# aquaskyline/Clairvoyante

Hardware: AMD Instinct MI355X
Metric: candidate tensors/sec (higher is better)
Workload: dtype f32

## Files before the change

clairvoyante_amd/csrc/cv_kernels_conv.hpp:

```cpp
#pragma once

template <int P, bool ACT = false>
__device__ __forceinline__ unsigned pool_code4(const f4 (&older)[P > 1 ? P - 1 : 1], f4 v, f4 o)
{
    unsigned c = 0;
#pragma unroll
    for (int r = 0; r < 4; r++) {
        int idx = P - 1;
#pragma unroll
        for (int d = P - 2; d >= 0; d--) {
            bool hit = older[d][r] == o[r];
            if constexpr (ACT) hit = hit && __builtin_signbit(older[d][r]) == __builtin_signbit(o[r]);
            idx = hit ? d : idx;
        }
        (void)v;
        c |= (unsigned)idx << (4 * r);
    }
    return c;
}

template <int POOL, bool SAVE = false>
__global__ __launch_bounds__(256) void conv1_tm(const float *__restrict__ x, int64_t n,
                                                 const float *__restrict__ wp1,
                                                 const float *__restrict__ bias, int cout,
                                                 f4 *__restrict__ out_tm, int G, u32x2 *__restrict__ code_tm = nullptr)
{
    constexpr int HIN = CV_INPUT_H, HOUT = HIN - POOL + 1, SPLIT = 4;
    const int lane = threadIdx.x & 63;
    const int wv = blockIdx.x * 4 + (threadIdx.x >> 6);
    const int g = wv / SPLIT, part = wv % SPLIT;
    if (g >= G) return;
    const int r0 = (HOUT * part) / SPLIT, r1 = (HOUT * (part + 1)) / SPLIT;
    const int c = lane & 15, q = lane >> 4;
    int64_t cand = (int64_t)g * 16 + c;
    if (cand >= n) cand = n - 1;
    const float *xp = x + (size_t)cand * (HIN * 16) + q;
    float A[4];
#pragma unroll
    for (int kw = 0; kw < 4; kw++) A[kw] = wp1[kw * 64 + lane];
    const f4 b4 = load_bias4(bias, 0, q, cout);
    f4 pw[POOL > 1 ? POOL - 1 : 1][4];
#pragma unroll
    for (int j = 0; j < (POOL > 1 ? POOL - 1 : 1); j++)
#pragma unroll
        for (int w = 0; w < 4; w++) pw[j][w] = (f4){0.f, 0.f, 0.f, 0.f};
    float xw[4], xn[4];
#pragma unroll
    for (int w = 0; w < 4; w++) xw[w] = xp[r0 * 16 + w * 4];
    f4 *op = out_tm + (size_t)g * HOUT * 4 * 64 + lane;
    const int hend = r1 + POOL - 1;
#pragma unroll 1
    for (int h = r0; h < hend; h++) {
        {
            const int hn = h + 1 < hend ? h + 1 : h;
#pragma unroll
            for (int w = 0; w < 4; w++) xn[w] = xp[hn * 16 + w * 4];
        }
        f4 acc[4];
#pragma unroll
        for (int w = 0; w < 4; w++) acc[w] = (f4){0.f, 0.f, 0.f, 0.f};
#pragma unroll
        for (int kw = 0; kw < 4; kw++)
#pragma unroll
            for (int wo = 0; wo < 4; wo++) {
                const int wi = wo + kw - 1;
                if (wi < 0 || wi > 3) continue;
                acc[wo] = mfma4(A[kw], xw[wi], acc[wo]);
            }
        if constexpr (!SAVE && POOL > 1) {
#pragma unroll
            for (int w = 0; w < 4; w++) {
                const f4 t = acc[w] + b4;
                const f4 o = max4(pw[POOL - 2][w], t);
#pragma unroll
                for (int j = POOL - 2; j > 0; j--) pw[j][w] = max4(pw[j - 1][w], t);
                pw[0][w] = t;
                if (h - r0 >= POOL - 1) op[(size_t)((h - (POOL - 1)) * 4 + w) * 64] = selu4(o);
            }
#pragma unroll
            for (int w = 0; w < 4; w++) xw[w] = xn[w];
            continue;
        }
        f4 v[4];
#pragma unroll
        for (int w = 0; w < 4; w++) v[w] = selu4(acc[w] + b4);
        if constexpr (POOL > 1) {
            f4 o[4];
#pragma unroll
            for (int w = 0; w < 4; w++) {
                o[w] = v[w];
#pragma unroll
                for (int j = 0; j < POOL - 1; j++) o[w] = max4(o[w], pw[j][w]);
            }
            if constexpr (SAVE) {
                if (h - r0 >= POOL - 1) {
                    unsigned cw[4];
#pragma unroll
                    for (int w = 0; w < 4; w++) {
                        f4 older[POOL - 1];
#pragma unroll
                        for (int j = 0; j < POOL - 1; j++) older[j] = pw[j][w];
                        cw[w] = pool_code4<POOL, true>(older, v[w], o[w]);
                    }
                    code_tm[((size_t)g * HOUT + (h - (POOL - 1))) * 64 + lane] = (u32x2){cw[0] | (cw[1] << 16), cw[2] | (cw[3] << 16)};
                }
            }
#pragma unroll
            for (int j = 0; j + 1 < POOL - 1; j++)
#pragma unroll
                for (int w = 0; w < 4; w++) pw[j][w] = pw[j + 1][w];
#pragma unroll
            for (int w = 0; w < 4; w++) pw[POOL - 2][w] = v[w];
            if (h - r0 >= POOL - 1) {
#pragma unroll
                for (int w = 0; w < 4; w++) op[(size_t)((h - (POOL - 1)) * 4 + w) * 64] = o[w];
            }
        } else {
#pragma unroll
            for (int w = 0; w < 4; w++) op[(size_t)(h * 4 + w) * 64] = v[w];
        }
#pragma unroll
        for (int w = 0; w < 4; w++) xw[w] = xn[w];
    }
}

__device__ __forceinline__ f4 selu4_low(f4 v)
{
    const cvm::f2v a = cvm::selu2((cvm::f2v){v[0], v[1]});
    return (f4){a[0], a[1], 0.0f, 0.0f};
}

template <int FRONT, bool HALF = false>
struct front_source {
    static constexpr int NP = FRONT > 1 ? FRONT - 1 : 1;
    const float *xp;
    float A[4];
    f4 b4;
    f4 cw[NP][4];
    float xc[4], xn[4];
    int hx;

    __device__ __forceinline__ void load_x(float (&dst)[4], int h)
    {
        if (h < CV_INPUT_H) {
#pragma unroll
            for (int w = 0; w < 4; w++) dst[w] = xp[h * 16 + w * 4];
        }
    }
    __device__ __forceinline__ void conv1_row(f4 (&v)[4])
    {
        f4 acc[4];
#pragma unroll
        for (int w = 0; w < 4; w++) acc[w] = (f4){0.f, 0.f, 0.f, 0.f};
#pragma unroll
        for (int kw = 0; kw < 4; kw++)
#pragma unroll
            for (int wo = 0; wo < 4; wo++) {
                const int wi = wo + kw - 1;
                if (wi < 0 || wi > 3) continue;
                acc[wo] = mfma4(A[kw], xc[wi], acc[wo]);
            }
#pragma unroll
        for (int w = 0; w < 4; w++) v[w] = acc[w] + b4;
#pragma unroll
        for (int w = 0; w < 4; w++) xc[w] = xn[w];
        hx++;
        load_x(xn, hx + 1);
    }
    __device__ __forceinline__ void init(const float *x, int64_t cand, int q, const float *wp1,
                                         const float *bias1, int cout1, int lane, int h0 = 0)
    {
        xp = x + (size_t)cand * (CV_INPUT_H * 16) + q;
#pragma unroll
        for (int kw = 0; kw < 4; kw++) A[kw] = wp1[kw * 64 + lane];
        b4 = load_bias4(bias1, 0, q, cout1);
        hx = h0;
        load_x(xc, h0);
        load_x(xn, h0 + 1);
        if constexpr (FRONT > 1) {
#pragma unroll
            for (int r = 0; r < FRONT - 1; r++) {
                f4 v[4];
                conv1_row(v);
#pragma unroll
                for (int w = 0; w < 4; w++) {
#pragma unroll
                    for (int j = FRONT - 2; j > 0; j--) cw[j][w] = r == 0 ? v[w] : max4(cw[j - 1][w], v[w]);
                    cw[0][w] = v[w];
                }
            }
        }
    }
    __device__ __forceinline__ void next(f4 (&row)[4][1])
    {
        f4 v[4];
        conv1_row(v);
        if constexpr (FRONT > 1) {
#pragma unroll
            for (int w = 0; w < 4; w++) {
                const f4 o = max4(cw[FRONT - 2][w], v[w]);
#pragma unroll
                for (int j = FRONT - 2; j > 0; j--) cw[j][w] = max4(cw[j - 1][w], v[w]);
                cw[0][w] = v[w];
                row[w][0] = HALF ? selu4_low(o) : selu4(o);
            }
        } else {
#pragma unroll
            for (int w = 0; w < 4; w++) row[w][0] = HALF ? selu4_low(v[w]) : selu4(v[w]);
        }
    }
};

#define CV_CONV_XCD_UNITS(W) ((W) != 1 && (W) != 2 && (W) != 4)
template <int KH, int CINB, int NT, int POOL, int HIN, int FRONT, int MODE, int HSPLIT = 1, int KS4 = 4>
__global__ __launch_bounds__(256, 2) void conv_tm(const f4 *__restrict__ in_tm, const float *__restrict__ x,
                                                   int64_t n, const float *__restrict__ wp1,
                                                   const float *__restrict__ bias1, int cout1,
                                                   const f4 *__restrict__ wp, const float *__restrict__ bias,
                                                   int cout, f4 *__restrict__ out_tm, f4 *__restrict__ act_tm, int G,
                                                   int rows_per = 0)
{
    static_assert(FRONT == 0 || CINB == 1, "the fused first layer feeds one 16-channel fragment");
    static_assert(MODE != 2 || (POOL == 1 && FRONT == 0), "the data-gradient pass has no pooling / first layer");
    static_assert(HSPLIT >= 1 || FRONT == 0, "flat ranges read their rows from a TM buffer (position parts may make them: front_source::init h0)");
    static_assert(HSPLIT != 0 || (FRONT == 0 && (MODE != 0 || POOL == 1)), "flat ranges: training kernels, and inference layers without pooling (slim small passes)");
    extern __shared__ __attribute__((aligned(16))) f4 ldsw[];
    constexpr int PADT = MODE == 2 ? KH - 1 - (KH - 1) / 2 : (KH - 1) / 2;
    constexpr int PADL = MODE == 2 ? 2 : 1;
    constexpr int HOUT = HIN - POOL + 1;
    constexpr int NFRAG = NT * KH * 4 * CINB;
    for (int i = threadIdx.x; i < NFRAG * 64; i += 256) ldsw[i] = wp[i];
    __syncthreads();
    const int lane = threadIdx.x & 63;
    int wv = __builtin_amdgcn_readfirstlane(blockIdx.x * 4 + (threadIdx.x >> 6));
    if constexpr (HSPLIT >= 1 && CV_CONV_XCD_UNITS(NT * HSPLIT)) {
        if (gridDim.x >= 16) {
            const int x = blockIdx.x & 7;
            const int lw = __builtin_amdgcn_readfirstlane((blockIdx.x >> 3) * 4 + (threadIdx.x >> 6));
            wv = ((lw / (NT * HSPLIT)) * 8 + x) * (NT * HSPLIT) + lw % (NT * HSPLIT);
        }
    }
    constexpr int HSD = HSPLIT > 0 ? HSPLIT : 1;
    int nt, gF, gL, hs = 0, r0 = 0, r1 = 0;
    if constexpr (HSPLIT == 0) {
        nt = wv % NT;
        r0 = (wv / NT) * rows_per;
        r1 = r0 + rows_per < G * HOUT ? r0 + rows_per : G * HOUT;
        if (r0 >= r1) return;
        gF = r0 / HOUT; gL = (r1 - 1) / HOUT;
    } else {
        const int gt = wv / HSD;
        hs = wv % HSD; nt = gt % NT; gF = gL = gt / NT;
        if (gF >= G) return;
    }
    CV_STAMP_BEGIN
    const int q = lane >> 4;
    const f4 b4 = MODE == 2 ? (f4){0.f, 0.f, 0.f, 0.f} : load_bias4(bias, nt, q, cout);
    const f4 *wl = ldsw + (size_t)nt * (KH * 4 * CINB * 64) + lane;
#pragma unroll 1
    for (int g = gF; g <= gL; g++) {
    int hbeg, hend;
    if constexpr (HSPLIT == 0) {
        const int oa = r0 - g * HOUT > 0 ? r0 - g * HOUT : 0, ob = r1 - g * HOUT < HOUT ? r1 - g * HOUT : HOUT;
        hbeg = oa; hend = POOL > 1 ? ob + POOL - 1 : ob;
    } else {
        hbeg = POOL > 1 ? HOUT * hs / HSD : HIN * hs / HSD;
        hend = POOL > 1 ? HOUT * (hs + 1) / HSD + POOL - 1 : HIN * (hs + 1) / HSD;
    }
    const f4 *inp = in_tm + (size_t)g * (HIN * 4 * CINB * 64) + lane;
    f4 *op = out_tm + (size_t)g * (HOUT * 4 * NT * 64) + (size_t)nt * 64 + lane;

    front_source<FRONT, (KS4 <= 2)> fs;
    if constexpr (FRONT > 0) {
        int64_t cand = (int64_t)g * 16 + (lane & 15);
        if (cand >= n) cand = n - 1;
        fs.init(x, cand, q, wp1, bias1, cout1, lane, hbeg - PADT > 0 ? hbeg - PADT : 0);
    }
    auto fetch_row = [&](int hr, f4 (&row)[4][CINB]) {
        if constexpr (FRONT > 0) {
            fs.next(row);
        } else {
#pragma unroll
            for (int w = 0; w < 4; w++)
#pragma unroll
                for (int cb = 0; cb < CINB; cb++) row[w][cb] = inp[(size_t)((hr * 4 + w) * CINB + cb) * 64];
        }
    };
    constexpr bool SPREAD = FRONT == 0;
    static_assert(CINB <= 3, "the counted wait below names at most 12 fragments");
    const f4 *const inp_s = in_tm + (size_t)__builtin_amdgcn_readfirstlane(g) * (HIN * 4 * CINB * 64);
    const unsigned lane16 = (unsigned)lane * 16u;
    auto load_piece = [&](int hr, int w, int cb, f4 &dst) {
        const f4 *ps = inp_s + (size_t)((hr * 4 + w) * CINB + cb) * 64;
        asm volatile("global_load_dwordx4 %0, %1, %2" : "=v"(dst) : "v"(lane16), "s"(ps));
    };

    f4 win[KH][4][CINB];
    f4 nxt[4][CINB];
    f4 pw[POOL > 1 ? POOL - 1 : 1][4];
    const f4 zero = (f4){0.f, 0.f, 0.f, 0.f};
#pragma unroll
    for (int j = 0; j < (POOL > 1 ? POOL - 1 : 1); j++)
#pragma unroll
        for (int w = 0; w < 4; w++) pw[j][w] = zero;
#pragma unroll
    for (int j = 0; j < KH; j++) {
        const int hr = hbeg + j - PADT;
        f4 tmp[4][CINB];
#pragma unroll
        for (int w = 0; w < 4; w++)
#pragma unroll
            for (int cb = 0; cb < CINB; cb++) tmp[w][cb] = zero;
        if (hr >= 0 && hr < HIN) fetch_row(hr, tmp);
#pragma unroll
        for (int w = 0; w < 4; w++)
#pragma unroll
            for (int cb = 0; cb < CINB; cb++) {
                if (j < KH - 1) win[j][w][cb] = tmp[w][cb]; else nxt[w][cb] = tmp[w][cb];
            }
    }
#pragma unroll 1
    for (int h = hbeg; h < hend; h++) {
#pragma unroll
        for (int w = 0; w < 4; w++)
#pragma unroll
            for (int cb = 0; cb < CINB; cb++) win[KH - 1][w][cb] = nxt[w][cb];
        {
            const int hr = h + 1 + (KH - 1) - PADT;
            if (!SPREAD && hr < HIN) fetch_row(hr, nxt);
        }
        const int hnext = h + 1 + (KH - 1) - PADT < HIN ? h + 1 + (KH - 1) - PADT : HIN - 1;
        f4 acc[4];
#pragma unroll
        for (int w = 0; w < 4; w++) acc[w] = zero;
#pragma unroll
        for (int kh = 0; kh < KH; kh++) {
            const int hr = h + kh - PADT;
            const bool on = hr >= 0 && hr < HIN;
            if (on) {
#pragma unroll
                for (int kw = 0; kw < 4; kw++)
#pragma unroll
                    for (int cb = 0; cb < CINB; cb++) {
                        const f4 A = wl[(size_t)((kh * 4 + kw) * CINB + cb) * 64];
#pragma unroll
                        for (int s = 0; s < KS4; s++)
#pragma unroll
                            for (int wo = 0; wo < 4; wo++) {
                                const int wi = wo + kw - PADL;
                                if (wi < 0 || wi > 3) continue;
                                acc[wo] = mfma4(A[s], win[kh][wi][cb][s], acc[wo]);
                            }
                        if constexpr (SPREAD) {
                            if (kh == 0) load_piece(hnext, kw, cb, nxt[kw][cb]);
                        }
                    }
            } else if (SPREAD && kh == 0) {
#pragma unroll
                for (int kw = 0; kw < 4; kw++)
#pragma unroll
                    for (int cb = 0; cb < CINB; cb++) load_piece(hnext, kw, cb, nxt[kw][cb]);
            }
        }
        if constexpr (SPREAD) {
            {
                if constexpr (CINB == 1)
                    asm volatile("s_waitcnt vmcnt(0)" : "+v"(nxt[0][0]), "+v"(nxt[1][0]), "+v"(nxt[2][0]), "+v"(nxt[3][0]) : : "memory");
                else if constexpr (CINB == 2)
                    asm volatile("s_waitcnt vmcnt(0)" : "+v"(nxt[0][0]), "+v"(nxt[1][0]), "+v"(nxt[2][0]), "+v"(nxt[3][0]),
                                 "+v"(nxt[0][1]), "+v"(nxt[1][1]), "+v"(nxt[2][1]), "+v"(nxt[3][1]) : : "memory");
                else
                    asm volatile("s_waitcnt vmcnt(0)" : "+v"(nxt[0][0]), "+v"(nxt[1][0]), "+v"(nxt[2][0]), "+v"(nxt[3][0]),
                                 "+v"(nxt[0][1]), "+v"(nxt[1][1]), "+v"(nxt[2][1]), "+v"(nxt[3][1]),
                                 "+v"(nxt[0][CINB - 1]), "+v"(nxt[1][CINB - 1]), "+v"(nxt[2][CINB - 1]), "+v"(nxt[3][CINB - 1]) : : "memory");
            }
        }
        if constexpr (MODE == 0 && POOL > 1) {
#pragma unroll
            for (int w = 0; w < 4; w++) {
                const f4 t = acc[w] + b4;
                const f4 o = max4(pw[POOL - 2][w], t);
#pragma unroll
                for (int j = POOL - 2; j > 0; j--) pw[j][w] = max4(pw[j - 1][w], t);
                pw[0][w] = t;
                if (h - hbeg >= POOL - 1) {
                    op[(size_t)((h - (POOL - 1)) * 4 + w) * (NT * 64)] = selu4(o);
                }
            }
#pragma unroll
            for (int j = 0; j + 1 < KH; j++)
#pragma unroll
                for (int w = 0; w < 4; w++)
#pragma unroll
                    for (int cb = 0; cb < CINB; cb++) win[j][w][cb] = win[j + 1][w][cb];
            continue;
        }
        f4 v[4];
        if constexpr (MODE == 2) {
#pragma unroll
            for (int w = 0; w < 4; w++) v[w] = acc[w];
            if (act_tm) {
                const f4 *yp = act_tm + (size_t)g * (HOUT * 4 * NT * 64) + (size_t)nt * 64 + lane;
#pragma unroll
                for (int w = 0; w < 4; w++) {
                    const f4 y = yp[(size_t)(h * 4 + w) * (NT * 64)];
#pragma unroll
                    for (int k = 0; k < 4; k++) v[w][k] *= cv_selu_grad_from_out(y[k]);
                }
            }
        } else {
#pragma unroll
            for (int w = 0; w < 4; w++) v[w] = selu4(acc[w] + b4);
        }
        if constexpr (POOL > 1) {
            f4 o[4];
#pragma unroll
            for (int w = 0; w < 4; w++) {
                o[w] = v[w];
#pragma unroll
                for (int j = 0; j < POOL - 1; j++) o[w] = max4(o[w], pw[j][w]);
            }
            if constexpr (MODE == 1) {
                if (h - hbeg >= POOL - 1) {
                    unsigned cw[4];
#pragma unroll
                    for (int w = 0; w < 4; w++) {
                        f4 older[POOL - 1];
#pragma unroll
                        for (int j = 0; j < POOL - 1; j++) older[j] = pw[j][w];
                        cw[w] = pool_code4<POOL, true>(older, v[w], o[w]);
                    }
                    u32x2 *cp = reinterpret_cast<u32x2 *>(act_tm);
                    cp[(((size_t)g * HOUT + (h - (POOL - 1))) * NT + nt) * 64 + lane] = (u32x2){cw[0] | (cw[1] << 16), cw[2] | (cw[3] << 16)};
                }
            }
#pragma unroll
            for (int j = 0; j + 1 < POOL - 1; j++)
#pragma unroll
                for (int w = 0; w < 4; w++) pw[j][w] = pw[j + 1][w];
#pragma unroll
            for (int w = 0; w < 4; w++) pw[POOL - 2][w] = v[w];
            if (h - hbeg >= POOL - 1) {
#pragma unroll
                for (int w = 0; w < 4; w++) op[(size_t)((h - (POOL - 1)) * 4 + w) * (NT * 64)] = o[w];
            }
        } else {
#pragma unroll
            for (int w = 0; w < 4; w++) op[(size_t)(h * 4 + w) * (NT * 64)] = v[w];
        }
#pragma unroll
        for (int j = 0; j + 1 < KH; j++)
#pragma unroll
            for (int w = 0; w < 4; w++)
#pragma unroll
                for (int cb = 0; cb < CINB; cb++) win[j][w][cb] = win[j + 1][w][cb];
    }
    }
    CV_STAMP_END(MODE == 2 && KH == 3 && CINB == 3, 2);
    CV_STAMP_END(MODE == 1 && KH == 2 && CINB == 1 && FRONT == 0, 6);
}

template <int CH, bool FLAT = false>
__global__ __launch_bounds__(FLAT ? 128 : 256, 2) void front2_tm(const float *__restrict__ x, int64_t n,
                                                     const float *__restrict__ wp1, const float *__restrict__ bias1,
                                                     int cout1, const f4 *__restrict__ wp,
                                                     const float *__restrict__ bias, int cout,
                                                     f4 *__restrict__ out_tm, int G, int rows_per = 0)
{
    constexpr int P1 = 5, H1 = CV_INPUT_H - P1 + 1;
    constexpr int NT = 2, P2 = 4, H2 = H1 - P2 + 1;
    constexpr int NW = NT * 2 * 4 * 64;
    extern __shared__ __attribute__((aligned(16))) f4 lds[];
    f4 *rows = lds + NW;
    for (int i = threadIdx.x; i < NW; i += (FLAT ? 128 : 256)) lds[i] = wp[i];
    const int lane = threadIdx.x & 63, wid = threadIdx.x >> 6;
    const int gl = FLAT ? 0 : wid >> 1, nt = wid & 1;
    int gF, gL, r0 = 0, r1 = 0;
    bool live = true;
    if constexpr (FLAT) {
        r0 = (int)blockIdx.x * rows_per;
        r1 = r0 + rows_per < G * H2 ? r0 + rows_per : G * H2;
        if (r0 >= r1) return;
        gF = r0 / H2; gL = (r1 - 1) / H2;
    } else {
        const int gq = blockIdx.x * 2 + gl;
        live = gq < G;
        gF = gL = live ? gq : G - 1;
    }
    const int q = lane >> 4;
    float A1[4];
#pragma unroll
    for (int kw = 0; kw < 4; kw++) A1[kw] = wp1[kw * 64 + lane];
    const f4 b1 = load_bias4(bias1, 0, q, cout1);
    const f4 b2 = load_bias4(bias, nt, q, cout);
    const f4 *wl = lds + (size_t)nt * (2 * 4 * 64) + lane;
    f4 *myrows = rows + (size_t)gl * (CH * 4 * 64) + lane;
    const f4 zero = (f4){0.f, 0.f, 0.f, 0.f};
    f4 prev[4], m1[4], m2[4], m3[4];
#pragma unroll
    for (int w = 0; w < 4; w++) { prev[w] = zero; m1[w] = zero; m2[w] = zero; m3[w] = zero; }
    __syncthreads();
    CV_PHASE_BEGIN
#pragma unroll 1
    for (int g = gF; g <= gL; g++) {
    int oa = 0, ob = H2;
    if constexpr (FLAT) {
        oa = r0 - g * H2 > 0 ? r0 - g * H2 : 0;
        ob = r1 - g * H2 < H2 ? r1 - g * H2 : H2;
    }
    const int pend = ob + P2 < H1 ? ob + P2 : H1;
    int64_t cand = (int64_t)g * 16 + (lane & 15);
    if (cand >= n) cand = n - 1;
    const float *xp = x + (size_t)cand * (CV_INPUT_H * 16) + q;
    f4 *op = out_tm + (size_t)g * (H2 * 4 * NT * 64) + (size_t)nt * 64 + lane;

    auto out_row = [&](int h, const f4 (&cur)[4], bool has_cur) {
        f4 acc[4];
#pragma unroll
        for (int w = 0; w < 4; w++) acc[w] = zero;
#pragma unroll
        for (int kw = 0; kw < 4; kw++) {
            const f4 A = wl[(size_t)(0 * 4 + kw) * 64];
#pragma unroll
            for (int s4 = 0; s4 < 4; s4++)
#pragma unroll
                for (int wo = 0; wo < 4; wo++) {
                    const int wi = wo + kw - 1;
                    if (wi < 0 || wi > 3) continue;
                    acc[wo] = mfma4(A[s4], prev[wi][s4], acc[wo]);
                }
        }
        if (has_cur) {
#pragma unroll
            for (int kw = 0; kw < 4; kw++) {
                const f4 A = wl[(size_t)(1 * 4 + kw) * 64];
#pragma unroll
                for (int s4 = 0; s4 < 4; s4++)
#pragma unroll
                    for (int wo = 0; wo < 4; wo++) {
                        const int wi = wo + kw - 1;
                        if (wi < 0 || wi > 3) continue;
                        acc[wo] = mfma4(A[s4], cur[wi][s4], acc[wo]);
                    }
            }
        }
#pragma unroll
        for (int w = 0; w < 4; w++) {
            const f4 t = acc[w] + b2;
            const f4 o = max4(m3[w], t);
            m3[w] = max4(m2[w], t);
            m2[w] = max4(m1[w], t);
            m1[w] = t;
            if (h - oa >= P2 - 1 && live) op[(size_t)((h - (P2 - 1)) * 4 + w) * (NT * 64)] = selu4(o);
        }
    };

#pragma unroll 1
    for (int c0 = oa; c0 < pend; c0 += CH) {
        const int cn = pend - c0 < CH ? pend - c0 : CH;
        const int half = (cn + 1) >> 1;
        const int a0 = c0 + nt * half;
        const int a1 = a0 + half < c0 + cn ? a0 + half : c0 + cn;
        if (a0 < a1) {
            static_assert(CH == 6, "the block pooling below is written for three rows per wave");
            constexpr int HALF = CH / 2, NRAW = HALF + P1 - 1;
            float xr[NRAW][4];
#pragma unroll
            for (int r = 0; r < NRAW; r++) {
                const int rr = a0 + r < CV_INPUT_H ? a0 + r : CV_INPUT_H - 1;
#pragma unroll
                for (int w = 0; w < 4; w++) xr[r][w] = xp[rr * 16 + w * 4];
            }
            CV_PHASE(0);
            CV_PHASE_DRAIN();
            CV_PHASE(3);
            f4 t[NRAW][4];
#pragma unroll
            for (int r = 0; r < NRAW; r++) {
                f4 acc[4];
#pragma unroll
                for (int w = 0; w < 4; w++) acc[w] = zero;
#pragma unroll
                for (int kw = 0; kw < 4; kw++)
#pragma unroll
                    for (int wo = 0; wo < 4; wo++) {
                        const int wi = wo + kw - 1;
                        if (wi < 0 || wi > 3) continue;
                        acc[wo] = mfma4(A1[kw], xr[r][wi], acc[wo]);
                    }
#pragma unroll
                for (int w = 0; w < 4; w++) t[r][w] = acc[w] + b1;
            }
#pragma unroll
            for (int w = 0; w < 4; w++) {
                const f4 c = max3_4(t[2][w], t[3][w], t[4][w]);
                const f4 o0 = max3_4(t[0][w], t[1][w], c);
                const f4 o1 = max3_4(t[1][w], c, t[5][w]);
                const f4 o2 = max3_4(c, t[5][w], t[6][w]);
                myrows[(size_t)((a0 - c0 + 0) * 4 + w) * 64] = selu4(o0);
                if (a0 + 1 < a1) myrows[(size_t)((a0 - c0 + 1) * 4 + w) * 64] = selu4(o1);
                if (a0 + 2 < a1) myrows[(size_t)((a0 - c0 + 2) * 4 + w) * 64] = selu4(o2);
            }
        }
        CV_PHASE(0);
        __syncthreads();
        CV_PHASE(2);
#pragma unroll 1
        for (int p = c0; p < c0 + cn; p++) {
            f4 cur[4];
#pragma unroll
            for (int w = 0; w < 4; w++) cur[w] = myrows[(size_t)((p - c0) * 4 + w) * 64];
            if (p > oa) out_row(p - 1, cur, true);
#pragma unroll
            for (int w = 0; w < 4; w++) prev[w] = cur[w];
        }
        CV_PHASE(1);
        __syncthreads();
        CV_PHASE(2);
    }
    if (ob == H2) out_row(H1 - 1, prev, false);
    }
    CV_PHASE(1);
    CV_PHASE_END(true, wid);
}

template <int CINB, int NT, int HIN, int WAVES, int MINW, bool SAVE = false>
__global__ __launch_bounds__(WAVES * 64, MINW) void conv3_rot(const f4 *__restrict__ in_tm, const f4 *__restrict__ wp,
                                                            const float *__restrict__ bias, int cout,
                                                            f4 *__restrict__ out_tm, int G, u32x2 *__restrict__ code_tm = nullptr,
                                                            int rows_per = 0)
{
    constexpr int KH = 3, PADT = 1, POOL = 3, HOUT = HIN - POOL + 1;
    extern __shared__ __attribute__((aligned(16))) f4 ldsw[];
    constexpr int NFRAG = NT * KH * 4 * CINB;
    for (int i = threadIdx.x; i < NFRAG * 64; i += WAVES * 64) ldsw[i] = wp[i];
    __syncthreads();
    const int lane = threadIdx.x & 63;
    int wv = __builtin_amdgcn_readfirstlane(blockIdx.x * WAVES + (threadIdx.x >> 6));
    const bool flat = rows_per > 0;
    if (gridDim.x >= 16) {
        const int x = blockIdx.x & 7;
        const int lw = __builtin_amdgcn_readfirstlane((blockIdx.x >> 3) * WAVES + (threadIdx.x >> 6));
        wv = ((lw / NT) * 8 + x) * NT + lw % NT;
    }
    const int nt = wv % NT;
    int gF = wv / NT, gL = gF, r0 = 0, r1 = 0;
    if (flat) {
        r0 = (wv / NT) * rows_per;
        r1 = r0 + rows_per < G * HOUT ? r0 + rows_per : G * HOUT;
        if (r0 >= r1) return;
        gF = r0 / HOUT; gL = (r1 - 1) / HOUT;
    } else if (gF >= G) return;
    CV_STAMP_BEGIN
    const int q = lane >> 4;
    const f4 b4 = load_bias4(bias, nt, q, cout);
    const f4 *wl = ldsw + (size_t)nt * (KH * 4 * CINB * 64) + lane;
    const f4 zero = (f4){0.f, 0.f, 0.f, 0.f};
    const unsigned lane16 = (unsigned)lane * 16u;
#pragma unroll 1
    for (int g = gF; g <= gL; g++) {
    int hbeg = 0, hend = HIN;
    if (flat) {
        hbeg = r0 - g * HOUT > 0 ? r0 - g * HOUT : 0;
        hend = (r1 - g * HOUT < HOUT ? r1 - g * HOUT : HOUT) + POOL - 1;
    }
    const f4 *inp = in_tm + (size_t)g * (HIN * 4 * CINB * 64) + lane;
    f4 *op = out_tm + (size_t)g * (HOUT * 4 * NT * 64) + (size_t)nt * 64 + lane;
    f4 win[3][4][CINB];
    f4 tp[3][4];
#pragma unroll
    for (int j = 0; j < 3; j++)
#pragma unroll
        for (int w = 0; w < 4; w++) tp[j][w] = zero;
    auto load_row = [&](int hr, f4 (&row)[4][CINB]) {
#pragma unroll
        for (int w = 0; w < 4; w++)
#pragma unroll
            for (int cb = 0; cb < CINB; cb++) row[w][cb] = inp[(size_t)((hr * 4 + w) * CINB + cb) * 64];
    };
    load_row(hbeg, win[1]);
    if (hbeg > 0) load_row(hbeg - 1, win[0]);
    static_assert(CINB == 2, "the counted wait below names 8 fragments");
    const f4 *const inp_s = in_tm + (size_t)g * (HIN * 4 * CINB * 64);
    auto load_piece = [&](int hr, int w, int cb, f4 &dst) {
        const f4 *ps = inp_s + (size_t)((hr * 4 + w) * CINB + cb) * 64;
        asm volatile("global_load_dwordx4 %0, %1, %2" : "=v"(dst) : "v"(lane16), "s"(ps));
    };
    auto step = [&](auto Rc, int h) {
        constexpr int R = decltype(Rc)::value;
        const int hnext = h + 1 < HIN ? h + 1 : HIN - 1;
        f4 acc[4];
#pragma unroll
        for (int w = 0; w < 4; w++) acc[w] = zero;
#pragma unroll
        for (int kh = 0; kh < KH; kh++) {
            const int hr = h + kh - PADT;
            const bool on = hr >= 0 && hr < HIN;
            if (kh == KH - 1) {
                f4 (&nw)[4][CINB] = win[(R + 2) % 3];
                asm volatile("s_waitcnt vmcnt(0)" : "+v"(nw[0][0]), "+v"(nw[1][0]), "+v"(nw[2][0]), "+v"(nw[3][0]),
                             "+v"(nw[0][1]), "+v"(nw[1][1]), "+v"(nw[2][1]), "+v"(nw[3][1]) : : "memory");
            }
            if (on) {
#pragma unroll
                for (int kw = 0; kw < 4; kw++)
#pragma unroll
                    for (int cb = 0; cb < CINB; cb++) {
                        const f4 A = wl[(size_t)((kh * 4 + kw) * CINB + cb) * 64];
#pragma unroll
                        for (int s = 0; s < 4; s++)
#pragma unroll
                            for (int wo = 0; wo < 4; wo++) {
                                const int wi = wo + kw - 1;
                                if (wi < 0 || wi > 3) continue;
                                acc[wo] = mfma4(A[s], win[(R + kh) % 3][wi][cb][s], acc[wo]);
                            }
                        if (kh == 0) load_piece(hnext, kw, cb, win[(R + 2) % 3][kw][cb]);
                    }
            } else if (kh == 0) {
#pragma unroll
                for (int kw = 0; kw < 4; kw++)
#pragma unroll
                    for (int cb = 0; cb < CINB; cb++) load_piece(hnext, kw, cb, win[(R + 2) % 3][kw][cb]);
            }
        }
#pragma unroll
        for (int w = 0; w < 4; w++) {
            if constexpr (SAVE) tp[R][w] = selu4(acc[w] + b4);
            else tp[R][w] = acc[w] + b4;
            if (h - hbeg >= POOL - 1) {
                if constexpr (SAVE) op[(size_t)((h - (POOL - 1)) * 4 + w) * (NT * 64)] = max3_4(tp[0][w], tp[1][w], tp[2][w]);
                else op[(size_t)((h - (POOL - 1)) * 4 + w) * (NT * 64)] = selu4(max3_4(tp[0][w], tp[1][w], tp[2][w]));
            }
        }
        if constexpr (SAVE) {
            if (h - hbeg >= POOL - 1) {
                unsigned cw[4];
#pragma unroll
                for (int w = 0; w < 4; w++) {
                    const f4 older[2] = {tp[(R + 1) % 3][w], tp[(R + 2) % 3][w]};
                    cw[w] = pool_code4<3, true>(older, tp[R][w], max3_4(tp[0][w], tp[1][w], tp[2][w]));
                }
                code_tm[(((size_t)g * HOUT + (h - (POOL - 1))) * NT + nt) * 64 + lane] = (u32x2){cw[0] | (cw[1] << 16), cw[2] | (cw[3] << 16)};
            }
        }
    };
#pragma unroll 1
    for (int h0 = hbeg; h0 < hend; h0 += 3) {
        step(std::integral_constant<int, 0>{}, h0);
        __builtin_amdgcn_sched_barrier(0);
        if (h0 + 1 < hend) step(std::integral_constant<int, 1>{}, h0 + 1);
        __builtin_amdgcn_sched_barrier(0);
        if (h0 + 2 < hend) step(std::integral_constant<int, 2>{}, h0 + 2);
        __builtin_amdgcn_sched_barrier(0);
    }
    }
    CV_STAMP_END(SAVE, 1);
}
```

clairvoyante_amd/csrc/cv_math.hpp:

```cpp
#pragma once
#include <hip/hip_runtime.h>
#include <stdint.h>

namespace cvm {

__device__ __forceinline__ float bits2f(uint32_t u) { return __builtin_bit_cast(float, u); }

__device__ __forceinline__ float expf_fixed(float x)
{
    if (x != x) return x;
    if (x > 88.72283905206835f) return __builtin_inff();
    if (x < -87.33654475055310f) return 0.0f;
    float z = __builtin_rintf(x * 1.44269504088896341f);
    float r = __builtin_fmaf(z, -0.693359375f, x);
    r = __builtin_fmaf(z, 2.12194440e-4f, r);
    float r2 = r * r;
    float p = 1.9875691500e-4f;
    p = __builtin_fmaf(p, r, 1.3981999507e-3f);
    p = __builtin_fmaf(p, r, 8.3334519073e-3f);
    p = __builtin_fmaf(p, r, 4.1665795894e-2f);
    p = __builtin_fmaf(p, r, 1.6666665459e-1f);
    p = __builtin_fmaf(p, r, 5.0000001201e-1f);
    float y = __builtin_fmaf(p, r2, r);
    y = y + 1.0f;
    int n = (int)z;
    int n1 = n >> 1, n2 = n - n1;
    y = y * bits2f((uint32_t)(n1 + 127) << 23);
    y = y * bits2f((uint32_t)(n2 + 127) << 23);
    return y;
}

constexpr float SELU_ALPHA = 1.6732632423543772848170429916717f;
constexpr float SELU_SCALE = 1.0507009873554804934193349852946f;

constexpr float SELU_SA = (float)(1.0507009873554804934193349852946 * 1.6732632423543772848170429916717);

__device__ __forceinline__ float selu(float x)
{
    const float xc = __builtin_amdgcn_fmed3f(x, -87.33654475055310f, 0.0f);
    float z = __builtin_rintf(xc * 1.44269504088896341f);
    float r = __builtin_fmaf(z, -0.69314718055994530942f, xc);
    float r2 = r * r;
    float p = 1.9875691500e-4f;
    p = __builtin_fmaf(p, r, 1.3981999507e-3f);
    p = __builtin_fmaf(p, r, 8.3334519073e-3f);
    p = __builtin_fmaf(p, r, 4.1665795894e-2f);
    p = __builtin_fmaf(p, r, 1.6666665459e-1f);
    p = __builtin_fmaf(p, r, 5.0000001201e-1f);
    float y = __builtin_fmaf(p, r2, r);
    y = y + 1.0f;
    y = __builtin_ldexpf(y, (int)z);
    const float mag = __builtin_fmaf(y, -SELU_SA, SELU_SA);
    const float pos = SELU_SCALE * x;
    return x < 0.0f ? -mag : __builtin_fabsf(pos);
}

typedef float f2v __attribute__((ext_vector_type(2)));

__device__ __forceinline__ f2v selu2(f2v x)
{
    f2v xc;
    xc[0] = __builtin_amdgcn_fmed3f(x[0], -87.33654475055310f, 0.0f);
    xc[1] = __builtin_amdgcn_fmed3f(x[1], -87.33654475055310f, 0.0f);
    const f2v t = xc * 1.44269504088896341f;
    f2v z;
    z[0] = __builtin_rintf(t[0]); z[1] = __builtin_rintf(t[1]);
    const f2v r = __builtin_elementwise_fma(z, (f2v)(-0.69314718055994530942f), xc);
    const f2v r2 = r * r;
    f2v p = (f2v)(1.9875691500e-4f);
    p = __builtin_elementwise_fma(p, r, (f2v)(1.3981999507e-3f));
    p = __builtin_elementwise_fma(p, r, (f2v)(8.3334519073e-3f));
    p = __builtin_elementwise_fma(p, r, (f2v)(4.1665795894e-2f));
    p = __builtin_elementwise_fma(p, r, (f2v)(1.6666665459e-1f));
    p = __builtin_elementwise_fma(p, r, (f2v)(5.0000001201e-1f));
    f2v y = __builtin_elementwise_fma(p, r2, r);
    y = y + 1.0f;
    y[0] = __builtin_ldexpf(y[0], (int)z[0]);
    y[1] = __builtin_ldexpf(y[1], (int)z[1]);
    const f2v mag = __builtin_elementwise_fma(y, (f2v)(-SELU_SA), (f2v)(SELU_SA));
    const f2v pos = SELU_SCALE * x;
    f2v o;
    o[0] = x[0] < 0.0f ? -mag[0] : __builtin_fabsf(pos[0]);
    o[1] = x[1] < 0.0f ? -mag[1] : __builtin_fabsf(pos[1]);
    return o;
}

__device__ __forceinline__ float selu_grad(float pre)
{
    if (pre >= 0.0f) return SELU_SCALE;
    return SELU_SCALE * (SELU_ALPHA * expf_fixed(pre));
}

__device__ __forceinline__ float sigmoid(float x) { return 1.0f / (1.0f + expf_fixed(-x)); }

template <int N>
__device__ __forceinline__ void softmax(const float (&l)[N], float (&p)[N])
{
    float m = l[0];
#pragma unroll
    for (int i = 1; i < N; i++) m = fmaxf(m, l[i]);
    float s = 0.0f;
#pragma unroll
    for (int i = 0; i < N; i++) {
        p[i] = expf_fixed(l[i] - m);
        s = (i == 0) ? p[0] : s + p[i];
    }
#pragma unroll
    for (int i = 0; i < N; i++) p[i] = p[i] / s;
}

}
```

clairvoyante_amd/csrc/cv_tile.hpp:

```cpp
#pragma once
#include "cv_internal.hpp"
#include "cv_math.hpp"
#include "cv_unpool.hpp"
#include <type_traits>
#include <functional>
#include <atomic>
#include <string.h>

typedef float f4 __attribute__((ext_vector_type(4)));

#if defined(CV_WG_STAMP) && defined(CV_TILE_STAMPS)
constexpr int CV_STAMP_KERNELS = 8;
__device__ unsigned long long cv_wg_stamp[CV_STAMP_KERNELS * 4096 * 4];
__device__ unsigned cv_wg_stamp_n[CV_STAMP_KERNELS];
extern "C" int cv_debug_wg_stamps(unsigned long long *out, unsigned *counts)
{
    if (hipMemcpyFromSymbol(counts, HIP_SYMBOL(cv_wg_stamp_n), sizeof(cv_wg_stamp_n)) != hipSuccess) return 1;
    return hipMemcpyFromSymbol(out, HIP_SYMBOL(cv_wg_stamp), sizeof(cv_wg_stamp)) != hipSuccess;
}
struct cv_stamp {
    unsigned long long t0, c0;
    __device__ __forceinline__ cv_stamp() : t0(__builtin_amdgcn_s_memrealtime()), c0(__builtin_amdgcn_s_memtime()) {}
    __device__ __forceinline__ void end(int kid) const
    {
        asm volatile("s_waitcnt vmcnt(0)" ::: "memory");
        const unsigned long long t1 = __builtin_amdgcn_s_memrealtime(), c1 = __builtin_amdgcn_s_memtime();
        const unsigned hw = __builtin_amdgcn_s_getreg(4 | (31 << 11)), xcc = __builtin_amdgcn_s_getreg(20 | (31 << 11));
        if ((threadIdx.x & 63) == 0) {
            const unsigned i = atomicAdd(&cv_wg_stamp_n[kid], 1u) & 4095u;
            unsigned long long *o = cv_wg_stamp + ((size_t)kid * 4096 + i) * 4;
            o[0] = t0; o[1] = t1; o[2] = c1 - c0; o[3] = ((unsigned long long)xcc << 32) | hw;
        }
    }
};
#define CV_STAMP_BEGIN const cv_stamp cv_st;
#define CV_STAMP_END(cond, kid) do { if (cond) cv_st.end(kid); } while (0)
#ifdef CV_ROW_PHASES
#define CV_PHASE_BEGIN unsigned long long cv_ph[4] = {0, 0, 0, 0}; unsigned long long cv_pt = __builtin_amdgcn_s_memtime();
#define CV_PHASE(i) do { const unsigned long long t_ = __builtin_amdgcn_s_memtime(); cv_ph[i] += t_ - cv_pt; cv_pt = t_; } while (0)
#define CV_PHASE_END(cond, w) do { if ((cond) && (threadIdx.x & 63) == 0) { const unsigned i_ = atomicAdd(&cv_wg_stamp_n[7], 1u) & 4095u; \
    unsigned long long *o_ = cv_wg_stamp + ((size_t)7 * 4096 + i_) * 4; o_[0] = cv_ph[0]; o_[1] = cv_ph[1]; o_[2] = cv_ph[2]; o_[3] = (unsigned long long)(w) | (cv_ph[3] << 8); } } while (0)
#define CV_PHASE_DRAIN() asm volatile("s_waitcnt vmcnt(0)" ::: "memory")
#endif
#else
#define CV_STAMP_BEGIN
#define CV_STAMP_END(cond, kid) do { } while (0)
#endif
#ifndef CV_PHASE_BEGIN
#define CV_PHASE_BEGIN
#define CV_PHASE(i) do { } while (0)
#define CV_PHASE_END(cond, w) do { } while (0)
#endif
#ifndef CV_PHASE_DRAIN
#define CV_PHASE_DRAIN() do { } while (0)
#endif

namespace {

__device__ __forceinline__ f4 mfma4(float a, float b, f4 c)
{
    return __builtin_amdgcn_mfma_f32_16x16x4f32(a, b, c, 0, 0, 0);
}

__device__ __forceinline__ f4 selu4(f4 v)
{
    const cvm::f2v a = cvm::selu2((cvm::f2v){v[0], v[1]}), b = cvm::selu2((cvm::f2v){v[2], v[3]});
    return (f4){a[0], a[1], b[0], b[1]};
}

__device__ __forceinline__ float vmaxf(float a, float b)
{
    float r;
    asm("v_max_f32 %0, %1, %2" : "=v"(r) : "v"(a), "v"(b));
    return r;
}

__device__ __forceinline__ f4 max3_4(f4 a, f4 b, f4 c)
{
    f4 r;
#pragma unroll
    for (int k = 0; k < 4; k++) {
        float v;
        asm("v_max3_f32 %0, %1, %2, %3" : "=v"(v) : "v"(a[k]), "v"(b[k]), "v"(c[k]));
        r[k] = v;
    }
    return r;
}

__device__ __forceinline__ f4 max4(f4 a, f4 b)
{
    f4 r;
    r[0] = vmaxf(a[0], b[0]); r[1] = vmaxf(a[1], b[1]); r[2] = vmaxf(a[2], b[2]); r[3] = vmaxf(a[3], b[3]);
    return r;
}

__device__ __forceinline__ f4 load_bias4(const float *__restrict__ bias, int ob, int q, int nout)
{
    f4 b;
#pragma unroll
    for (int r = 0; r < 4; r++) {
        int f = 16 * ob + 4 * r + q;
        b[r] = f < nout ? bias[f] : 0.0f;
    }
    return b;
}

typedef unsigned int u32x2 __attribute__((ext_vector_type(2)));

struct cv_dropout_args { float *d4, *amask; int nunits; float rate; uint64_t seed, step; int64_t cand0; };

__device__ __forceinline__ void dropout_value(float &v, float &mk, int unit, int nunits, int64_t cand, float rate, uint64_t seed,
                                              uint64_t step, uint64_t salt = 0)
{
    mk = 1.0f;
    if (unit >= nunits) { v = 0.0f; mk = 0.0f; }
    else if (rate > 0.0f) {
        const float ap = -1.7580993408473766f;
        float q = 1.0f - rate;
        float a = sqrtf(1.0f / (q * ((1.0f - q) * (ap * ap) + 1.0f)));
        float b = 0.0f - a * ((1.0f - q) * ap);
        uint64_t ctr = (seed * 0x9E3779B97F4A7C15ull) ^ (step << 40) ^ (uint64_t)(cand * nunits + unit) ^ salt;
        ctr += 0x9E3779B97F4A7C15ull;
        ctr = (ctr ^ (ctr >> 30)) * 0xBF58476D1CE4E5B9ull;
        ctr = (ctr ^ (ctr >> 27)) * 0x94D2049BB133111Bull;
        ctr = ctr ^ (ctr >> 31);
        float u = (float)((uint32_t)(ctr >> 32) >> 8) * (1.0f / 16777216.0f);
        float keep = floorf(q + u);
        v = a * (v * keep + ap * (1.0f - keep)) + b;
        mk = a * keep;
    }
}

inline unsigned nblk(int64_t total, int bs) { return (unsigned)((total + bs - 1) / bs); }

template <typename K>
int set_lds(K kernel, size_t bytes)
{
    CV_HIP(hipFuncSetAttribute(reinterpret_cast<const void *>(kernel),
                               hipFuncAttributeMaxDynamicSharedMemorySize, (int)bytes));
    return 0;
}

bool arch_is(const cv_arch &a, int k0, int k1, int k2, int c0, int c1, int c2, int p0, int p1, int p2,
             int f4_, int f5_)
{
    return a.kh[0] == k0 && a.kh[1] == k1 && a.kh[2] == k2 && a.cout[0] == c0 && a.cout[1] == c1 &&
           a.cout[2] == c2 && a.pool[0] == p0 && a.pool[1] == p1 && a.pool[2] == p2 && a.fc4 == f4_ &&
           a.fc5 == f5_;
}

static inline bool is_full(const cv_arch &a) { return arch_is(a, 1, 2, 3, 16, 32, 48, 5, 4, 3, 336, 168); }
static inline bool is_slim(const cv_arch &a) { return arch_is(a, 1, 3, 5, 8, 16, 32, 1, 1, 1, 36, 18); }

static int device_cus(int *out)
{
    static std::atomic<int> cus_by_dev[64];
    int dev = 0;
    CV_HIP(hipGetDevice(&dev));
    int cus = cus_by_dev[dev & 63].load(std::memory_order_relaxed);
    if (cus == 0) {
        CV_HIP(hipDeviceGetAttribute(&cus, hipDeviceAttributeMultiprocessorCount, dev));
        if (cus <= 0) cus = 256;
        cus_by_dev[dev & 63].store(cus, std::memory_order_relaxed);
    }
    *out = cus;
    return 0;
}

}
```

Baseline: 18.65 million.

## Batch SELU evaluation and restructure pool-4 sliding max in fused conv1/conv2

Adds a batched SELU routine that evaluates several f4 vectors at once with an interleaved polynomial exp, keeping constants in registers, so independent lanes can hide latency. The conv2 pooling window of four rows is rewritten as a two-slot ping-pong of partial maxima using max3, which cuts the per-row max chain. The row loop is unrolled by two so the slot index is a compile-time constant. This adds code size and register pressure and uses a custom exp approximation whose accuracy may differ slightly from the previous selu.

```diff
diff --git a/clairvoyante_amd/csrc/cv_kernels_conv.hpp b/clairvoyante_amd/csrc/cv_kernels_conv.hpp
--- a/clairvoyante_amd/csrc/cv_kernels_conv.hpp
+++ b/clairvoyante_amd/csrc/cv_kernels_conv.hpp
@@ -496,9 +496,10 @@
     const f4 *wl = lds + (size_t)nt * (2 * 4 * 64) + lane;
     f4 *myrows = rows + (size_t)gl * (CH * 4 * 64) + lane;
     const f4 zero = (f4){0.f, 0.f, 0.f, 0.f};
-    f4 prev[4], m1[4], m2[4], m3[4];
-#pragma unroll
-    for (int w = 0; w < 4; w++) { prev[w] = zero; m1[w] = zero; m2[w] = zero; m3[w] = zero; }
+    const cvm::selu_consts sk = cvm::selu_make_consts();
+    f4 ra[4], rb[4], tq[2][4], pm[2][4];
+#pragma unroll
+    for (int w = 0; w < 4; w++) { ra[w] = zero; rb[w] = zero; tq[0][w] = zero; tq[1][w] = zero; pm[0][w] = zero; pm[1][w] = zero; }
     __syncthreads();
     CV_PHASE_BEGIN
 #pragma unroll 1
@@ -514,7 +515,8 @@
     const float *xp = x + (size_t)cand * (CV_INPUT_H * 16) + q;
     f4 *op = out_tm + (size_t)g * (H2 * 4 * NT * 64) + (size_t)nt * 64 + lane;
 
-    auto out_row = [&](int h, const f4 (&cur)[4], bool has_cur) {
+    auto out_row = [&](auto Sc, int h, const f4 (&prev)[4], const f4 (&cur)[4], bool has_cur) {
+        constexpr int S = decltype(Sc)::value;
         f4 acc[4];
 #pragma unroll
         for (int w = 0; w < 4; w++) acc[w] = zero;
@@ -544,17 +546,21 @@
                     }
             }
         }
+        f4 o[4];
 #pragma unroll
         for (int w = 0; w < 4; w++) {
-            const f4 t = acc[w] + b2;
-            const f4 o = max4(m3[w], t);
-            m3[w] = max4(m2[w], t);
-            m2[w] = max4(m1[w], t);
-            m1[w] = t;
-            if (h - oa >= P2 - 1 && live) op[(size_t)((h - (P2 - 1)) * 4 + w) * (NT * 64)] = selu4(o);
+            tq[S][w] = acc[w] + b2;
+            o[w] = max3_4(tq[S][w], tq[S ^ 1][w], pm[S][w]);
+            pm[S][w] = max4(tq[S][w], tq[S ^ 1][w]);
+        }
+        if (h - oa >= P2 - 1 && live) {
+            selu4xN(o, sk);
+#pragma unroll
+            for (int w = 0; w < 4; w++) op[(size_t)((h - (P2 - 1)) * 4 + w) * (NT * 64)] = o[w];
         }
     };
 
+    int last_slot = 1;
 #pragma unroll 1
     for (int c0 = oa; c0 < pend; c0 += CH) {
         const int cn = pend - c0 < CH ? pend - c0 : CH;
@@ -591,34 +597,72 @@
 #pragma unroll
                 for (int w = 0; w < 4; w++) t[r][w] = acc[w] + b1;
             }
+            f4 o0[4], o1[4], o2[4];
 #pragma unroll
             for (int w = 0; w < 4; w++) {
                 const f4 c = max3_4(t[2][w], t[3][w], t[4][w]);
-                const f4 o0 = max3_4(t[0][w], t[1][w], c);
-                const f4 o1 = max3_4(t[1][w], c, t[5][w]);
-                const f4 o2 = max3_4(c, t[5][w], t[6][w]);
-                myrows[(size_t)((a0 - c0 + 0) * 4 + w) * 64] = selu4(o0);
-                if (a0 + 1 < a1) myrows[(size_t)((a0 - c0 + 1) * 4 + w) * 64] = selu4(o1);
-                if (a0 + 2 < a1) myrows[(size_t)((a0 - c0 + 2) * 4 + w) * 64] = selu4(o2);
+                o0[w] = max3_4(t[0][w], t[1][w], c);
+                o1[w] = max3_4(t[1][w], c, t[5][w]);
+                o2[w] = max3_4(c, t[5][w], t[6][w]);
+            }
+            selu4xN(o0, sk);
+#pragma unroll
+            for (int w = 0; w < 4; w++) myrows[(size_t)((a0 - c0 + 0) * 4 + w) * 64] = o0[w];
+            if (a0 + 1 < a1) {
+                selu4xN(o1, sk);
+#pragma unroll
+                for (int w = 0; w < 4; w++) myrows[(size_t)((a0 - c0 + 1) * 4 + w) * 64] = o1[w];
+            }
+            if (a0 + 2 < a1) {
+                selu4xN(o2, sk);
+#pragma unroll
+                for (int w = 0; w < 4; w++) myrows[(size_t)((a0 - c0 + 2) * 4 + w) * 64] = o2[w];
             }
         }
         CV_PHASE(0);
         __syncthreads();
         CV_PHASE(2);
+        int p = c0;
+        if (c0 == oa) {
+            if (cn >= 2) {
+#pragma unroll
+                for (int w = 0; w < 4; w++) rb[w] = myrows[(size_t)w * 64];
+#pragma unroll
+                for (int w = 0; w < 4; w++) ra[w] = myrows[(size_t)(4 + w) * 64];
+                out_row(std::integral_constant<int, 1>{}, p, rb, ra, true);
+                p += 2;
+            } else {
+#pragma unroll
+                for (int w = 0; w < 4; w++) ra[w] = myrows[(size_t)w * 64];
+                p++;
+            }
+        }
 #pragma unroll 1
-        for (int p = c0; p < c0 + cn; p++) {
-            f4 cur[4];
-#pragma unroll
-            for (int w = 0; w < 4; w++) cur[w] = myrows[(size_t)((p - c0) * 4 + w) * 64];
-            if (p > oa) out_row(p - 1, cur, true);
-#pragma unroll
-            for (int w = 0; w < 4; w++) prev[w] = cur[w];
+        for (; p + 1 < c0 + cn; p += 2) {
+#pragma unroll
+            for (int w = 0; w < 4; w++) rb[w] = myrows[(size_t)((p - c0) * 4 + w) * 64];
+            out_row(std::integral_constant<int, 0>{}, p - 1, ra, rb, true);
+#pragma unroll
+            for (int w = 0; w < 4; w++) ra[w] = myrows[(size_t)((p + 1 - c0) * 4 + w) * 64];
+            out_row(std::integral_constant<int, 1>{}, p, rb, ra, true);
+        }
+        last_slot = 1;
+        if (p < c0 + cn) {
+            last_slot = 0;
+#pragma unroll
+            for (int w = 0; w < 4; w++) rb[w] = myrows[(size_t)((p - c0) * 4 + w) * 64];
+            out_row(std::integral_constant<int, 0>{}, p - 1, ra, rb, true);
+#pragma unroll
+            for (int w = 0; w < 4; w++) ra[w] = rb[w];
         }
         CV_PHASE(1);
         __syncthreads();
         CV_PHASE(2);
     }
-    if (ob == H2) out_row(H1 - 1, prev, false);
+    if (ob == H2) {
+        if (last_slot == 0) out_row(std::integral_constant<int, 1>{}, H1 - 1, ra, ra, false);
+        else out_row(std::integral_constant<int, 0>{}, H1 - 1, ra, ra, false);
+    }
     }
     CV_PHASE(1);
     CV_PHASE_END(true, wid);
diff --git a/clairvoyante_amd/csrc/cv_math.hpp b/clairvoyante_amd/csrc/cv_math.hpp
--- a/clairvoyante_amd/csrc/cv_math.hpp
+++ b/clairvoyante_amd/csrc/cv_math.hpp
@@ -85,6 +85,62 @@
     return o;
 }
 
+struct selu_consts { f2v p0, sa; };
+
+__device__ __forceinline__ selu_consts selu_make_consts()
+{
+    selu_consts k = {(f2v)(1.9875691500e-4f), (f2v)(SELU_SA)};
+    asm volatile("" : "+v"(k.p0), "+v"(k.sa));
+    return k;
+}
+
+template <int N>
+__device__ __forceinline__ void selu2xN(f2v (&x)[N], const selu_consts &k)
+{
+    f2v xc[N], z[N], r[N], r2[N], p[N], y[N];
+#pragma unroll
+    for (int i = 0; i < N; i++) {
+        xc[i][0] = __builtin_amdgcn_fmed3f(x[i][0], -87.33654475055310f, 0.0f);
+        xc[i][1] = __builtin_amdgcn_fmed3f(x[i][1], -87.33654475055310f, 0.0f);
+    }
+#pragma unroll
+    for (int i = 0; i < N; i++) z[i] = xc[i] * 1.44269504088896341f;
+#pragma unroll
+    for (int i = 0; i < N; i++) { z[i][0] = __builtin_rintf(z[i][0]); z[i][1] = __builtin_rintf(z[i][1]); }
+#pragma unroll
+    for (int i = 0; i < N; i++) r[i] = __builtin_elementwise_fma(z[i], (f2v)(-0.69314718055994530942f), xc[i]);
+#pragma unroll
+    for (int i = 0; i < N; i++) p[i] = __builtin_elementwise_fma(k.p0, r[i], (f2v)(1.3981999507e-3f));
+#pragma unroll
+    for (int i = 0; i < N; i++) r2[i] = r[i] * r[i];
+#pragma unroll
+    for (int i = 0; i < N; i++) p[i] = __builtin_elementwise_fma(p[i], r[i], (f2v)(8.3334519073e-3f));
+#pragma unroll
+    for (int i = 0; i < N; i++) p[i] = __builtin_elementwise_fma(p[i], r[i], (f2v)(4.1665795894e-2f));
+#pragma unroll
+    for (int i = 0; i < N; i++) p[i] = __builtin_elementwise_fma(p[i], r[i], (f2v)(1.6666665459e-1f));
+#pragma unroll
+    for (int i = 0; i < N; i++) p[i] = __builtin_elementwise_fma(p[i], r[i], (f2v)(5.0000001201e-1f));
+#pragma unroll
+    for (int i = 0; i < N; i++) y[i] = __builtin_elementwise_fma(p[i], r2[i], r[i]);
+#pragma unroll
+    for (int i = 0; i < N; i++) y[i] = y[i] + 1.0f;
+#pragma unroll
+    for (int i = 0; i < N; i++) {
+        y[i][0] = __builtin_ldexpf(y[i][0], (int)z[i][0]);
+        y[i][1] = __builtin_ldexpf(y[i][1], (int)z[i][1]);
+    }
+#pragma unroll
+    for (int i = 0; i < N; i++) y[i] = __builtin_elementwise_fma(y[i], (f2v)(-SELU_SA), k.sa);
+#pragma unroll
+    for (int i = 0; i < N; i++) r[i] = SELU_SCALE * x[i];
+#pragma unroll
+    for (int i = 0; i < N; i++) {
+        x[i][0] = x[i][0] < 0.0f ? -y[i][0] : __builtin_fabsf(r[i][0]);
+        x[i][1] = x[i][1] < 0.0f ? -y[i][1] : __builtin_fabsf(r[i][1]);
+    }
+}
+
 __device__ __forceinline__ float selu_grad(float pre)
 {
     if (pre >= 0.0f) return SELU_SCALE;
diff --git a/clairvoyante_amd/csrc/cv_tile.hpp b/clairvoyante_amd/csrc/cv_tile.hpp
--- a/clairvoyante_amd/csrc/cv_tile.hpp
+++ b/clairvoyante_amd/csrc/cv_tile.hpp
@@ -66,6 +66,17 @@
 {
     const cvm::f2v a = cvm::selu2((cvm::f2v){v[0], v[1]}), b = cvm::selu2((cvm::f2v){v[2], v[3]});
     return (f4){a[0], a[1], b[0], b[1]};
+}
+
+template <int NF>
+__device__ __forceinline__ void selu4xN(f4 (&v)[NF], const cvm::selu_consts &k)
+{
+    cvm::f2v x[2 * NF];
+#pragma unroll
+    for (int i = 0; i < NF; i++) { x[2 * i] = (cvm::f2v){v[i][0], v[i][1]}; x[2 * i + 1] = (cvm::f2v){v[i][2], v[i][3]}; }
+    cvm::selu2xN<2 * NF>(x, k);
+#pragma unroll
+    for (int i = 0; i < NF; i++) v[i] = (f4){x[2 * i][0], x[2 * i][1], x[2 * i + 1][0], x[2 * i + 1][1]};
 }
 
 __device__ __forceinline__ float vmaxf(float a, float b)
```

New measurement: 18.72 million (median of 6 runs). About the same (+0.4%).
